# numamma/numamma

Hardware: AMD Instinct MI355X
Metric: PEBS samples/s analysed (device-resident) (higher is better)
Workload: dtype u64

## Files before the change

numamma_amd/csrc/nmg_route.hip:

```cpp
#include <algorithm>

#include "nmg_device.h"
#include "nmg_route.h"

namespace nmg {

static_assert((uint64_t)kItemChunks * kChunk * kLaneMaxWeight < (1ull << kPackShift), "packed weight per item");


struct XRec {
  uint64_t addr, ts, w;
  uint64_t loc;
  uint32_t th, acc;
  bool esc;
  __device__ __forceinline__ uint32_t g(const XLayout& xl) const { return uint32_t(loc >> xl.obits); }
  __device__ __forceinline__ uint32_t off(const XLayout& xl) const {
    return uint32_t(loc & ((1ull << xl.obits) - 1)) << 3;
  }
};

__device__ __forceinline__ uint4 x_encode(const XLayout& xl, uint64_t pb, uint64_t addr, uint64_t ts, uint64_t w,
                                          uint32_t g, uint32_t off, uint32_t th, uint32_t acc) {
  const uint64_t ar = addr - pb, tr = ts - xl.tbase;
  const bool fit = (ar >> kAddrBits) == 0 && ts >= xl.tbase && (tr >> kTsBits) == 0 && w < xl.wesc;
// ... 652 lines not shown
      }
      rt_stamp<TIMING>(rt, 5);
      bool staged = false, counts = false;
      if (__ballot(lined)) {
        lid &= kLwLineMask;
        const uint32_t j = (uint32_t)dst & 3u, S = lw_s(lw), ahead = (lid - S) & kLwLineMask;
        counts = lined && !(lw & kLwBroken) && ahead < ahead_max;
        staged = counts && ahead == 0 && dst != ~0ull;
        if (lined && !(lw & kLwBroken) && ahead >= ahead_max) atomicOr(&s_lw[X.q], kLwBroken);
        if (staged) {
          s_line[X.q * 4 + j] = X.a;
          s_ldst[X.q] = (uint32_t)(dst >> 2);
        }
        __builtin_amdgcn_fence(__ATOMIC_RELEASE, "workgroup", "local");
        LineWord o = 0;
        if (counts)
          o = atomicAdd(&s_lw[X.q], (kLwOne << (3 * (lid & (kLwAhead - 1)))) +
                                        (staged ? kLwOne << (kLwMaskShift + j) : LineWord(0)));
        const bool done = counts && lw_count(o, lid) == 3 && lw_s(o) == lid;
        const uint32_t dmask = counts ? lw_mask(o) | (staged ? 1u << j : 0u) : 0u;
        if (TIMING) rt.acc[8] += (uint64_t)__popcll(__ballot(counts && !staged));
        const uint64_t dm = __ballot(done);
        if (dm) {
          if (done)
            s_tab[wave][__popcll(dm & ((1ull << lane) - 1))] =
                make_uint2(X.q | (dmask << 11) | (lid << 16), (uint32_t)(dst >> 2));
          __builtin_amdgcn_fence(__ATOMIC_RELEASE, "wavefront", "local");
          __builtin_amdgcn_wave_barrier();
          __builtin_amdgcn_fence(__ATOMIC_ACQUIRE, "wavefront", "local");
          const uint32_t nd = (uint32_t)__popcll(dm);
          auto piece_done = [&](uint2 t, uint32_t k) {
            __builtin_amdgcn_fence(__ATOMIC_RELEASE, "workgroup", "local");
            if (k == 0) {
              const uint32_t tq = t.x & 2047u;
              uint32_t l = t.x >> 16, m = (t.x >> 11) & 15u;
              while (true) {
                const LineWord ow = atomicAdd(&s_lw[tq], (kLwOne << kLwSShift) - (LineWord(4) << (3 * (l & (kLwAhead - 1)))) -
                                                            (LineWord(m) << kLwMaskShift));
                l = (l + 1) & kLwLineMask;
                if (lw_count(ow, l) != 4) break;
                m = 0;
              }
            }
          };
          for (uint32_t j0 = 0; j0 < nd; j0 += 16) {
            const uint32_t jj = j0 + ((uint32_t)lane >> 2);
            if (jj < nd) {
              const uint2 t = s_tab[wave][jj];
              const uint32_t tq = t.x & 2047u, tm = (t.x >> 11) & 15u, k = lane & 3;
              if ((tm >> k) & 1) rec16[uint64_t(t.y) * 4 + k] = rec16_of(s_line[tq * 4 + k]);
              piece_done(t, k);
            }
          }
          __builtin_amdgcn_fence(__ATOMIC_RELEASE, "wavefront", "local");
          __builtin_amdgcn_wave_barrier();
          __builtin_amdgcn_fence(__ATOMIC_ACQUIRE, "wavefront", "local");
        }
      }
      rt_stamp<TIMING>(rt, 9);
      const bool straight = dst != ~0ull && !counts;
      const bool alone = straight || (counts && !staged && dst != ~0ull);
      if (alone) rec16[dst] = rec16_of(X.a);
      if (TIMING) {
        rt.acc[6] += (uint64_t)__popcll(__ballot(staged));
        rt.acc[7] += (uint64_t)__popcll(__ballot(straight));
      }
      if (__ballot(ovf)) {
        if (ovf) {
          const uint64_t pbq = s_pb[X.q];
          const uint32_t o = atomicAdd(rp.ovf_cnt, 1u);
          if (o < rp.ovf_cap) {
            rp.ovf16[o] = X.a;
            rp.ovfx[o] = pbq;
          } else {
            XRec xr = x_decode(rp.xl, pbq, X.a);
            if (xr.esc) x_resolve(xr, rp.xl, p.data, p.sbufs);
            direct_attribute<TL>(p, xr.addr, xr.ts, xr.w, xr.th, xr.acc, X.lvl, rp.seq0 + xr.g(rp.xl), xr.off(rp.xl),
                             xr.g(rp.xl));
          }
        }
        vm_drain();
      }
      rt_stamp<TIMING>(rt, 10);
    };

    XF X;
    do {
      front(ra, rb, X);
      back(X);
      front(rb, ra, X);
      back(X);
    } while (d0.pad != kNoBuf);

    if (TIMING && lane == 0) {
      unsigned long long* o = p.dbg + (uint64_t(blockIdx.x) * (kWG / 64) + tid / 64) * kRouteTimingWords;
      for (int k = 0; k < 9; k++) o[k] = rt.acc[k];
      o[9] = nwin;
      uint32_t nb = 0;
      if (wave == 0)
        for (uint32_t q = 0; q < nlp; q++) nb += (s_lw[q] & kLwBroken) ? 1u : 0u;
      o[10] = nb;
      o[11] = rt.acc[9];
      o[12] = rt.acc[10];
    }
  }
  racc_drain(gacc[0], s_gsums[0], lane);
  racc_drain(gacc[1], s_gsums[1], lane);
  lds_sync();
#pragma unroll
  for (uint32_t a = 0; a < 2; a++) {
    if (tid < (int)kGlobalSums && s_gsums[a][tid])
      atomicAdd(reinterpret_cast<unsigned long long*>(p.sum64 + gsum_index(a, tid)), s_gsums[a][tid]);
    if (tid < (int)kBuckets && s_gsums[a][3 + 2 * tid]) {
      atomicMin(reinterpret_cast<unsigned long long*>(p.min64 + a * kBuckets + tid), s_gmins[a][tid]);
      atomicMax(reinterpret_cast<unsigned long long*>(p.max64 + a * kBuckets + tid), s_gmaxs[a][tid]);
    }
  }
  for (uint32_t q = tid; q < P; q += kR2WG) {
    const unsigned long long st = s_state[q];
    const uint32_t f = st_cnt(st), cu = st_cur(st), nx = st_next(st);
    if (cu == kStNone) continue;
    if (cu != kStOvf) rp.cmeta[c0 + cu] = q | (min(f, kChunk) << 24);
    if (nx != kStOvf) rp.cmeta[c0 + nx] = q | ((f > kChunk ? f - kChunk : 0u) << 24);
    if (q < nlp) {
      const uint32_t m = lw_mask(s_lw[q]);
      for (uint32_t j = 0; j < 4; j++)
        if ((m >> j) & 1u) rec16[uint64_t(s_ldst[q]) * 4 + j] = rec16_of(s_line[q * 4 + j]);
    }
  }
  if (tid == 0) rp.used[blockIdx.x] = min(s_taken, capl);
}


__global__ __launch_bounds__(256) void overflow_kernel(RouteParams rp) {
  const uint32_t n = min(*rp.ovf_cnt, rp.ovf_cap);
  for (uint32_t i = blockIdx.x * 256 + threadIdx.x; i < n; i += gridDim.x * 256) {
    XRec xr = x_decode(rp.xl, rp.ovfx[i], rp.ovf16[i]);
    if (xr.esc) x_resolve(xr, rp.xl, rp.p.data, rp.p.sbufs);
    const uint32_t lvl = ((rp.p.flags & NMG_F_OBJECT_LEVELS) || rp.p.cost)
                             ? raw_mem_lvl(rp.p.data, rp.p.sbufs[xr.g(rp.xl)].offset + xr.off(rp.xl))
                             : 0u;
    direct_attribute<true>(rp.p, xr.addr, xr.ts, xr.w, xr.th, xr.acc, lvl, rp.seq0 + xr.g(rp.xl), xr.off(rp.xl),
                     xr.g(rp.xl));
  }
}


__global__ __launch_bounds__(kWG) void count_kernel(CountParams cp) {
  __shared__ uint32_t s_cnt[kMaxParts + 1];
  const ScatterParams& r = cp.sc;
  const uint32_t tid = threadIdx.x, w = blockIdx.x, P = r.nparts;
  for (uint32_t q = tid; q < P; q += kWG) s_cnt[q] = 0;
  __syncthreads();
  const uint32_t c0 = r.chunk0[w], n = r.used[w];
  constexpr uint32_t kU = 8;
  for (uint32_t b = 0; b < n; b += kU * kWG) {
    uint32_t m[kU];
#pragma unroll
    for (uint32_t u = 0; u < kU; u++) {
      const uint32_t i = b + u * kWG + tid;
      m[u] = i < n ? r.cmeta[c0 + i] : 0u;
    }
#pragma unroll
    for (uint32_t u = 0; u < kU; u++)
      if (m[u] >> 24) atomicAdd(&s_cnt[m[u] & 0xffffffu], 1u);
  }
  __syncthreads();
  uint32_t* out = const_cast<uint32_t*>(r.pcnt) + uint64_t(w) * P;
  for (uint32_t q = tid; q < P; q += kWG) out[q] = s_cnt[q];
}

constexpr uint32_t kPlanRowGroups = kWG / 64;
__global__ __launch_bounds__(kWG) void plan_cols_kernel(PlanParams r) {
  __shared__ uint32_t s_sum[kPlanRowGroups][64];
  const uint32_t tid = threadIdx.x, c = tid & 63, rg = tid >> 6;
  const uint32_t P = r.nparts, q = blockIdx.x * 64 + c;
  const uint32_t per = (r.grid + kPlanRowGroups - 1) / kPlanRowGroups, w0 = rg * per;
  constexpr uint32_t kU = 16;
  uint32_t sum = 0;
  for (uint32_t b = 0; b < per; b += kU) {
    uint32_t v[kU];
#pragma unroll
    for (uint32_t u = 0; u < kU; u++) {
      const uint32_t w = w0 + b + u;
      v[u] = (q < P && b + u < per && w < r.grid) ? r.pcnt[uint64_t(w) * P + q] : 0u;
    }
#pragma unroll
    for (uint32_t u = 0; u < kU; u++) sum += v[u];
  }
  s_sum[rg][c] = sum;
  __syncthreads();
  uint32_t run = 0;
  for (uint32_t g = 0; g < rg; g++) run += s_sum[g][c];
  for (uint32_t b = 0; b < per; b += kU) {
    uint32_t v[kU];
#pragma unroll
    for (uint32_t u = 0; u < kU; u++) {
      const uint32_t w = w0 + b + u;
      v[u] = (q < P && b + u < per && w < r.grid) ? r.pcnt[uint64_t(w) * P + q] : 0u;
    }
#pragma unroll
    for (uint32_t u = 0; u < kU; u++) {
      const uint32_t w = w0 + b + u;
      if (q < P && b + u < per && w < r.grid) r.pcnt[uint64_t(w) * P + q] = run;
      run += v[u];
    }
  }
  if (q < P && rg == kPlanRowGroups - 1) r.pbase[q] = run;
}

__global__ __launch_bounds__(kWG) void plan_kernel(PlanParams r) {
  __shared__ uint32_t s_tot[kMaxParts + 1], s_nit[kMaxParts + 1], s_wsum[2][kWG / 64];
  const int tid = threadIdx.x, lane = tid & 63, wave = tid >> 6;
  const uint32_t P = r.nparts;
  for (uint32_t q = tid; q < P; q += kWG) {
    const uint32_t run = r.pbase[q];
    s_tot[q] = run;
    s_nit[q] = (run + kItemChunks - 1) / kItemChunks;
  }
  __syncthreads();
  const uint32_t i0 = 2 * (uint32_t)tid;
  const uint32_t t0 = i0 < P ? s_tot[i0] : 0u, t1 = i0 + 1 < P ? s_tot[i0 + 1] : 0u;
  const uint32_t n0 = i0 < P ? s_nit[i0] : 0u, n1 = i0 + 1 < P ? s_nit[i0 + 1] : 0u;
  uint32_t it = t0 + t1, in = n0 + n1;
#pragma unroll
  for (int o = 1; o < 64; o <<= 1) {
    const uint32_t a = __shfl_up(it, o, 64), b = __shfl_up(in, o, 64);
    if (lane >= o) {
      it += a;
      in += b;
    }
  }
  if (lane == 63) {
    s_wsum[0][wave] = it;
    s_wsum[1][wave] = in;
  }
  __syncthreads();
  uint32_t wt = 0, wn = 0;
  for (int w2 = 0; w2 < wave; w2++) {
    wt += s_wsum[0][w2];
    wn += s_wsum[1][w2];
  }
  const uint32_t tb = wt + it - (t0 + t1), nb = wn + in - (n0 + n1);
  for (uint32_t k = 0; k < 2; k++) {
    const uint32_t q = i0 + k;
    if (q >= P) break;
    const uint32_t base = tb + (k ? t0 : 0u), ibase = nb + (k ? n0 : 0u), tot = k ? t1 : t0;
    r.pbase[q] = base;
    for (uint32_t j = 0; j * kItemChunks < tot; j++)
      r.items[ibase + j] = make_uint4(q, base + j * kItemChunks, base + min(tot, (j + 1) * kItemChunks),
                                      tot <= kItemChunks ? 1u : 0u);
  }
  if (tid == kWG - 1) {
    r.ctl[0] = wn + in;
    r.ctl[1] = 0;
    r.ctl[3] = r.ctl[2];
    r.ctl[2] = 0;
  }
}

__global__ __launch_bounds__(kWG) void scatter_kernel(ScatterParams r) {
  __shared__ uint32_t s_cnt[kMaxParts + 1];
  const uint32_t tid = threadIdx.x, w = blockIdx.x, P = r.nparts;
  const uint32_t* off = r.pcnt + uint64_t(w) * P;
  for (uint32_t q = tid; q < P; q += kWG) s_cnt[q] = r.pbase[q] + off[q];
  __syncthreads();
  const uint32_t c0 = r.chunk0[w], n = r.used[w];
  const uint32_t pc = c0 >> r.pk;
  const uint32_t voff =
      (uint32_t)((reinterpret_cast<uint64_t>(r.pieces[pc]) - r.pool0) / (kChunk * sizeof(uint4))) - (pc << r.pk);
  constexpr uint32_t kU = 8;
  for (uint32_t b = 0; b < n; b += kU * kWG) {
    uint32_t m[kU];
#pragma unroll
    for (uint32_t u = 0; u < kU; u++) {
      const uint32_t i = b + u * kWG + tid;
      m[u] = i < n ? r.cmeta[c0 + i] : 0u;
    }
#pragma unroll
    for (uint32_t u = 0; u < kU; u++) {
      if (!(m[u] >> 24)) continue;
      const uint32_t k = atomicAdd(&s_cnt[m[u] & 0xffffffu], 1u);
      const uint32_t id = c0 + b + u * kWG + tid;
      r.clist[k] = make_uint2(id | ((m[u] >> 24) << kChunkIdBits), voff + id);
    }
  }
}


constexpr uint32_t kLWG = 1024;
constexpr int kLC = 2;

template <typename T>
__device__ __forceinline__ T l2_load(const T* p) {
  return __hip_atomic_load(p, __ATOMIC_RELAXED, __HIP_MEMORY_SCOPE_AGENT);
}

__device__ __forceinline__ void lds_pair(uint4& a, uint4& b) {
  asm volatile("" : "+v"(a.x), "+v"(a.y), "+v"(a.z), "+v"(a.w), "+v"(b.x), "+v"(b.y), "+v"(b.z), "+v"(b.w));
}
__device__ __forceinline__ void lds_pair(uint2& a, uint2& b) {
  asm volatile("" : "+v"(a.x), "+v"(a.y), "+v"(b.x), "+v"(b.y));
}

__device__ __forceinline__ uint64_t entry_id(const LocalParams& lp, uint32_t pos) {
  return lp.pe_ids ? lp.pe_ids[pos] : pos;
}

__device__ __forceinline__ int32_t match_older_pos(const Params& p, uint32_t first, uint32_t count, uint64_t addr,
                                                   uint64_t ts, uint64_t& baddr, uint64_t& hist) {
  for (uint32_t j = first + 1; j < first + count; j++) {
    const uint4* r = reinterpret_cast<const uint4*>(p.chain + j);
    const uint4 ra = r[0], rb = r[1];
    if (entry_match(ra, rb, addr, ts)) {
      const uint4 rc = r[2];
      baddr = u64of(ra.x, ra.y);
      hist = u64of(rc.x, rc.y);
      return (int32_t)j;
    }
  }
  return -1;
}

template <bool INSTR, bool PACKED, bool EXTRA>
__global__ __launch_bounds__(kLWG, 1) void local_kernel(LocalParams lp) {
  __shared__ uint64_t s_keys[kPartSlots];
  __shared__ uint4 s_pn[kPartSlots];
  __shared__ uint2 s_info[kPartSlots];
  __shared__ uint4 s_dir[kPartDir];
  __shared__ uint4 s_old[kOldLds];
  __shared__ uint32_t s_oinf[kOldLds];
  __shared__ unsigned long long s_owt[2][kPartEntries];
  __shared__ unsigned long long s_first[kPartEntries];
  __shared__ uint32_t s_pg[kPartCells / 2];
  __shared__ uint32_t s_clist[kItemChunks];
  __shared__ uint32_t s_item, s_cnext, s_nfound, s_big, s_took;
  __shared__ uint4 s_nx[4];
  __shared__ uint32_t s_coff[kItemChunks];

  Params& p = lp.p;
  const int tid = threadIdx.x, lane = tid & 63;
  const uint32_t nitems = lp.ctl[0];
  const uint32_t T = p.nb_threads;
  const bool pages = (p.flags & NMG_F_PAGE_HIST) != 0;
  RTimer rt;
#pragma unroll
  for (int k = 0; k < 12; k++) rt.acc[k] = 0;
  const bool tim = INSTR && (p.flags & kDbgLocalTiming) != 0;
  const bool nowork = INSTR && (p.flags & kDbgLocalNoWork) != 0, nosearch = INSTR && (p.flags & kDbgLocalNoSearch) != 0;
  const bool noobj = INSTR && (p.flags & kDbgLocalNoObj) != 0, nopage = INSTR && (p.flags & kDbgLocalNoPage) != 0;
  auto lstamp = [&](int i) {
    if (INSTR && tim) rt_stamp<true>(rt, i);
  };
  rt.last = tim ? stamp() : 0;
  uint32_t nchunks = 0, nit = 0;
  uint64_t textra = 0;
  uint32_t nfound = 0;
  if (tid == 0) s_nfound = 0;
  for (uint32_t i = tid; i < kPartEntries; i += kLWG) {
    s_owt[0][i] = s_owt[1][i] = 0;
    s_first[i] = ~0ull;
  }
  for (uint32_t i = tid; i < kPartCells / 2; i += kLWG) s_pg[i] = 0;
  static_assert(sizeof(PartInfo) == 48, "PartInfo: three uint4");
  auto take_next = [&]() {
    uint32_t idx = 0;
    if (lane == 0) idx = atomicAdd(lp.ctl + 1, 1u);
    idx = __builtin_amdgcn_readfirstlane(idx);
    if (lane == 0) s_item = idx;
    if (idx < nitems) {
      const uint4 nx = lp.items[idx];
      const uint32_t nq = __builtin_amdgcn_readfirstlane(nx.x);
      if (lane == 0) s_nx[0] = nx;
      if (lane < 3) s_nx[1 + lane] = reinterpret_cast<const uint4*>(lp.parts + nq)[lane];
    }
  };
  if (tid < 64) take_next();
  if (tid == 0) s_took = 0;
  while (true) {
    lds_sync();
    const uint32_t it = __builtin_amdgcn_readfirstlane(s_item);
    lstamp(6);
    if (it >= nitems) break;
    nit++;
    const uint4 item = s_nx[0];
    const uint32_t q = __builtin_amdgcn_readfirstlane(item.x);
    PartInfo pi;
    {
      uint4* pw = reinterpret_cast<uint4*>(&pi);
      pw[0] = s_nx[1];
      pw[1] = s_nx[2];
      pw[2] = s_nx[3];
    }
    const uint32_t dshift = __builtin_amdgcn_readfirstlane(pi.dshift);
    {
      static_assert(kPartKeys <= kLWG && kPartDir == kLWG && kOldLds <= kLWG, "one table element per thread");
      constexpr uint32_t kClPer = (kItemChunks + kLWG - 1) / kLWG;
      const uint32_t nk = pi.nk, nold = min(pi.ne - nk, kOldLds), ncl = item.z - item.y;
      uint64_t key = 0;
      uint4 pn = make_uint4(0, 0, 0, 0), od = pn;
      uint2 inf = make_uint2(0, 0);
      uint32_t oi = 0, cl[kClPer], cf[kClPer];
      if (tid < nk) {
        key = lp.pe_keys[uint64_t(q) * kPartSlots + tid];
        pn = lp.pe_pnode[uint64_t(q) * kPartSlots + tid];
        inf = lp.pe_info[uint64_t(q) * kPartSlots + tid];
      }
      const uint4 dd = lp.pe_dir[uint64_t(q) * kPartDir + tid];
      if (tid < nold) {
        od = lp.pe_old[uint64_t(q) * kOldLds + tid];
        oi = lp.pe_oinf[uint64_t(q) * kOldLds + tid];
      }
#pragma unroll
      for (uint32_t u = 0; u < kClPer; u++) {
        const uint2 ce = tid + u * kLWG < ncl ? lp.clist[item.y + tid + u * kLWG] : make_uint2(0u, 0u);
        cl[u] = ce.x;
        cf[u] = ce.y;
      }
      if (tid < nk) {
        s_keys[tid] = key;
        s_pn[tid] = pn;
        s_info[tid] = inf;
      }
      s_dir[tid] = dd;
      if (tid < nold) {
        s_old[tid] = od;
        s_oinf[tid] = oi;
      }
#pragma unroll
      for (uint32_t u = 0; u < kClPer; u++)
        if (tid + u * kLWG < ncl) {
          s_clist[tid + u * kLWG] = cl[u];
          s_coff[tid + u * kLWG] = cf[u];
        }
    }
    if (tid == 0) {
      s_cnext = 0;
      s_took = 0;
    }
    const uint32_t ncell = (pages && pi.pages_lds) ? T * pi.span : 0u;
    const bool excl = item.w != 0 && !(INSTR && (p.flags & kDbgLocalAtomics));
    if (tid == 0) s_big = 0;
    lds_sync();
    const uint64_t k0key = u64of(__builtin_amdgcn_readfirstlane((uint32_t)s_keys[0]),
                                 __builtin_amdgcn_readfirstlane((uint32_t)(s_keys[0] >> 32)));
    lstamp(7);

    const uint32_t nl = item.z - item.y;
    auto chunk_load = [&](uint32_t l, uint4& a) {
      const uint32_t e = l < nl ? s_coff[l] : 0u;
      a = lp.pool0[uint64_t(e) * kChunk + lane];
    };
    auto process = [&](uint32_t l0, const uint4 (&a16)[kLC]) {
      uint32_t li[kLC], cw[kLC];
      bool valid[kLC];
      uint64_t addr[kLC], ts[kLC], w[kLC];
      XRec xr[kLC];
#pragma unroll
      for (int j = 0; j < kLC; j++) {
        li[j] = l0 + j;
        cw[j] = s_clist[min(li[j], nl - 1)];
      }
#pragma unroll
      for (int j = 0; j < kLC; j++) valid[j] = (uint32_t)lane < (li[j] < nl ? cw[j] >> kChunkIdBits : 0u);
      if (INSTR && tim) {
        asm volatile("s_waitcnt vmcnt(2)" ::: "memory");
        nchunks += kLC;
      }
      lstamp(0);
      if (INSTR && nowork) {
#pragma unroll
        for (int j = 0; j < kLC; j++)
          if (lane == 0 && li[j] < nl)
            lp.cmatch[cw[j] & ((1u << kChunkIdBits) - 1)] = a16[j].x ^ a16[j].y ^ a16[j].z ^ a16[j].w;
        return;
      }
      bool esc = false;
#pragma unroll
      for (int j = 0; j < kLC; j++) {
        xr[j] = x_decode_rel(lp.xl, a16[j]);
        esc |= valid[j] && xr[j].esc;
      }
      if (__ballot(esc)) {
#pragma unroll
        for (int j = 0; j < kLC; j++)
          if (valid[j] && xr[j].esc) {
            x_resolve(xr[j], lp.xl, p.data, lp.descs);
            xr[j].addr -= k0key;
          }
        vm_drain();
      }
#pragma unroll
      for (int j = 0; j < kLC; j++) {
        addr[j] = xr[j].addr;
        ts[j] = xr[j].ts;
        w[j] = valid[j] ? xr[j].w : 0ull;
      }
      lstamp(1);
      uint32_t slot[kLC], sa[kLC], sn[kLC];
      uint4 de[kLC];
#pragma unroll
      for (int j = 0; j < kLC; j++)
        slot[j] = valid[j] ? (uint32_t)min(addr[j] >> dshift, (uint64_t)(kPartDir - 1)) : 0u;
#pragma unroll
      for (int j = 0; j < kLC; j++) de[j] = s_dir[slot[j]];
      static_assert(kLC == 2, "lds_pair: two chunks");
      lds_pair(de[0], de[1]);
#pragma unroll
      for (int j = 0; j < kLC; j++) {
        const uint32_t lo = de[j].x & 1023u, n = (de[j].x >> 10) & 2047u;
        const bool inl = n && ((de[j].x >> 21) & 1u);
        const uint64_t rs64 = addr[j] - (uint64_t(slot[j]) << dshift);
        const uint32_t rs = rs64 >> 16 ? 0x10000u : (uint32_t)rs64;
        const uint32_t c = (uint32_t)((de[j].y & 0xffffu) <= rs) + (uint32_t)((de[j].y >> 16) <= rs) +
                           (uint32_t)((de[j].z & 0xffffu) <= rs) + (uint32_t)((de[j].z >> 16) <= rs) +
                           (uint32_t)((de[j].w & 0xffffu) <= rs) + (uint32_t)((de[j].w >> 16) <= rs);
        const uint32_t a = inl ? lo + min(c, n) : lo;
        const uint32_t m = !inl ? n : (c == kDirInline && n > kDirInline) ? n - kDirInline : 0u;
        sa[j] = valid[j] ? a : 0u;
        sn[j] = valid[j] ? m : 0u;
      }
      if (INSTR && tim) {
#pragma unroll
        for (int j = 0; j < kLC; j++) rt.acc[11] += (uint64_t)__popcll(__ballot(sn[j] != 0));
      }
      {
        bool more = false;
#pragma unroll
        for (int j = 0; j < kLC; j++) more |= sn[j] != 0;
        while (more) {
          uint32_t half[kLC];
          uint64_t key[kLC];
#pragma unroll
          for (int j = 0; j < kLC; j++) {
            half[j] = (sn[j] + 1) >> 1;
            key[j] = s_keys[sa[j] + half[j]];
          }
          more = false;
#pragma unroll
          for (int j = 0; j < kLC; j++) {
            const bool le = key[j] - k0key <= addr[j];
            sa[j] += le ? half[j] : 0u;
            sn[j] = le ? sn[j] - half[j] : half[j] - (uint32_t)(sn[j] != 0);
            more |= sn[j] != 0;
          }
        }
      }
      if (INSTR && tim) {
        bool any = false;
#pragma unroll
        for (int j = 0; j < kLC; j++) any |= valid[j];
        (void)__builtin_amdgcn_readfirstlane(__ballot(any));
      }
      lstamp(2);
      const uint32_t (&r)[kLC] = sa;
      int32_t erel[kLC];
      uint64_t pofs[kLC];
      uint32_t hrel[kLC], pnw[kLC], tq[kLC];
      bool older[kLC], amb[kLC];
      {
        uint4 pn[kLC];
        uint2 inf[kLC];
#pragma unroll
        for (int j = 0; j < kLC; j++) {
          pn[j] = s_pn[r[j]];
          inf[j] = s_info[r[j]];
        }
        lds_pair(pn[0], pn[1]);
        lds_pair(inf[0], inf[1]);
#pragma unroll
        for (int j = 0; j < kLC; j++) {
          tq[j] = __builtin_amdgcn_alignbit((uint32_t)(ts[j] >> 32), (uint32_t)ts[j], kPnQShift);
          const bool live = valid[j] & !(INSTR && nosearch);
          const bool in = (addr[j] >= (uint64_t)inf[j].y) & (addr[j] < (uint64_t)pn[j].x);
          amb[j] = live & (xr[j].esc | ((pn[j].w & kPnExact) != 0) | (in & ((tq[j] == pn[j].y) | (tq[j] == pn[j].z))));
          const bool hit = live & !amb[j] & in & (tq[j] > pn[j].y) & (tq[j] < pn[j].z);
          erel[j] = hit ? (int32_t)(pn[j].w & 2047u) : -1;
          pofs[j] = hit ? addr[j] - inf[j].y : 0ull;
          hrel[j] = hit ? inf[j].x : kEmpty32;
          older[j] = live & !amb[j] & !hit & ((pn[j].w & kPnOlder) != 0);
          pnw[j] = live ? pn[j].w : 0u;
        }
      }
      bool anyamb = false;
#pragma unroll
      for (int j = 0; j < kLC; j++) {
        anyamb |= amb[j];
        if (INSTR && tim) rt.acc[10] +=(uint64_t)__popcll(__ballot(amb[j]));
      }
      if (__ballot(anyamb)) {
#pragma unroll
        for (int j = 0; j < kLC; j++) {
          if (!amb[j]) continue;
          const uint64_t fa = k0key + addr[j], ft = xr[j].esc ? ts[j] : lp.xl.tbase + ts[j];
          const uint4* gq = lp.pe_nodes + (uint64_t(q) * kPartSlots + (uint32_t)r[j]) * 2;
          const uint4 na = gq[0], nb = gq[1];
          if (entry_match(na, nb, fa, ft)) {
            erel[j] = (int32_t)(s_pn[r[j]].w & 2047u);
            pofs[j] = fa - u64of(na.x, na.y);
            hrel[j] = s_info[r[j]].x;
          } else {
            older[j] = (s_pn[r[j]].w & kPnOlder) != 0;
          }
        }
        vm_drain();
      }
      bool anyold = false;
#pragma unroll
      for (int j = 0; j < kLC; j++) anyold |= older[j];
      if (__ballot(anyold)) {
#pragma unroll
        for (int j = 0; j < kLC; j++) {
          if (!older[j] || xr[j].esc || !(pnw[j] & kPnOldLds)) continue;
          const uint32_t e = pnw[j] & 2047u, base = e - (uint32_t)r[j], c = (pnw[j] >> kPnOldShift) & 2047u;
          bool glob = false;
          for (uint32_t i = 0; i < c; i++) {
            const uint4 o = s_old[base + i];
            const bool in = addr[j] >= (uint64_t)o.w && addr[j] < (uint64_t)o.x;
            if (in && (tq[j] == o.y || tq[j] == o.z)) {
              glob = true;
              break;
            }
            if (in && tq[j] > o.y && tq[j] < o.z) {
              erel[j] = (int32_t)(e + 1 + i);
              pofs[j] = addr[j] - o.w;
              hrel[j] = s_oinf[base + i];
              break;
            }
          }
          older[j] = glob;
        }
        anyold = false;
#pragma unroll
        for (int j = 0; j < kLC; j++) anyold |= older[j];
      }
      if (__ballot(anyold)) {
#pragma unroll
        for (int j = 0; j < kLC; j++) {
          if (!older[j]) continue;
          const uint64_t fa = k0key + addr[j], ft = xr[j].esc ? ts[j] : lp.xl.tbase + ts[j];
          const uint4 d = reinterpret_cast<const uint4*>(p.nodes + pi.k0 + (uint32_t)r[j])[3];
          uint64_t hist = kHistSparse, baddr = 0;
          const int32_t pos = match_older_pos(p, d.y, d.x, fa, ft, baddr, hist);
          if (pos >= 0) {
            erel[j] = pos - (int32_t)pi.e0;
            pofs[j] = fa - baddr;
            hrel[j] = hist == kHistSparse ? kEmpty32
                      : PACKED && pi.cmap != ~0u ? lp.pe_lrel[pos]
                                         : (uint32_t)(hist - pi.cb);
          }
        }
        vm_drain();
      }
      {
        uint64_t mine = 0;
        uint32_t ml = 0, mc = 0;
#pragma unroll
        for (int j = 0; j < kLC; j++) {
          const uint64_t fm = __ballot(erel[j] >= 0);
          nfound += (uint32_t)__popcll(fm);
          mine = lane == j ? fm : mine;
          ml = lane == j ? li[j] : ml;
          mc = lane == j ? cw[j] : mc;
        }
        if (lane < kLC && ml < nl) lp.cmatch[mc & ((1u << kChunkIdBits) - 1)] = mine;
      }
      lstamp(3);
#pragma unroll
      for (int j = 0; j < kLC; j++) {
        bool ok = erel[j] >= 0 && !noobj && w[j] < kLaneMaxWeight;
        if (ok) atomicAdd(&s_owt[xr[j].acc][erel[j]], (1ull << kPackShift) | w[j]);
      }
      bool anybig = false;
#pragma unroll
      for (int j = 0; j < kLC; j++) anybig |= erel[j] >= 0 && w[j] >= kLaneMaxWeight;
      if (__ballot(anybig) && !noobj) {
        if (lane == 0) s_big = 1;
#pragma unroll
        for (int j = 0; j < kLC; j++) {
          if (erel[j] < 0 || w[j] < kLaneMaxWeight) continue;
          const uint64_t e = entry_id(lp, pi.e0 + (uint32_t)erel[j]);
          atomicAdd(reinterpret_cast<unsigned long long*>(p.sum64 + objcw_index(e, xr[j].acc, 0, p.nb_entries)), 1ull);
          atomicAdd(reinterpret_cast<unsigned long long*>(p.sum64 + objcw_index(e, xr[j].acc, 1, p.nb_entries)),
                    (unsigned long long)w[j]);
        }
        vm_drain();
      }
      if (!noobj) {
        unsigned long long cur[kLC];
#pragma unroll
        for (int j = 0; j < kLC; j++) cur[j] = s_first[erel[j] >= 0 ? erel[j] : 0];
#pragma unroll
        for (int j = 0; j < kLC; j++)
          if (erel[j] >= 0 && xr[j].loc < cur[j]) atomicMin(&s_first[erel[j]], (unsigned long long)xr[j].loc);
      }
      lstamp(4);
      if (pages && !nopage) {
        uint32_t page[kLC];
        bool glob = false;
#pragma unroll
        for (int j = 0; j < kLC; j++) {
          page[j] = uint32_t(int(pofs[j] / kPageSize));
          if (erel[j] >= 0 && hrel[j] != kEmpty32 && ncell) {
            const uint32_t c = xr[j].th * pi.span + hrel[j] + page[j], sh = 16 * (c & 1);
            atomicAdd(&s_pg[c >> 1], 1u << sh);
          }
          glob |= erel[j] >= 0 && (hrel[j] == kEmpty32 || !ncell);
        }
        if (__ballot(glob)) {
#pragma unroll
          for (int j = 0; j < kLC; j++) {
            if (erel[j] < 0) continue;
            if (hrel[j] != kEmpty32 && !ncell) {
              atomicAdd(p.hist + uint64_t(xr[j].th) * p.hist_cells + pi.cb + hrel[j] + page[j], 1u);
            } else if (hrel[j] == kEmpty32) {
              const uint32_t sidx = p.entries[entry_id(lp, pi.e0 + (uint32_t)erel[j])].sidx;
              if (sidx != ~0u)
                sparse_add(p, sparse_key(sidx, xr[j].th, page[j]), lp.seq0 + xr[j].g(lp.xl), xr[j].off(lp.xl), 1u);
            }
          }
          vm_drain();
        }
      }
      lstamp(5);
      if (EXTRA) {
        const bool lev = (p.flags & NMG_F_OBJECT_LEVELS) != 0;
        const bool tlon = p.tl != nullptr;
        const bool cost = p.cost != nullptr;
        bool need[kLC], any = false;
#pragma unroll
        for (int j = 0; j < kLC; j++) {
          need[j] = valid[j] && (p.smatch != nullptr || ((lev || tlon || cost) && erel[j] >= 0));
          any |= need[j];
        }
        if (__ballot(any)) {
          uint64_t eid[kLC];
          uint32_t lvl[kLC];
          bool row[kLC];
#pragma unroll
          for (int j = 0; j < kLC; j++) {
            eid[j] = 0;
            lvl[j] = 0;
            row[j] = false;
            if (!need[j]) continue;
            const uint64_t pos = lp.descs[xr[j].g(lp.xl)].offset + xr[j].off(lp.xl);
            const bool hit = erel[j] >= 0;
            if (hit) eid[j] = entry_id(lp, pi.e0 + (uint32_t)erel[j]);
            if (p.smatch) p.smatch[pos >> 3] = hit ? (uint32_t)eid[j] + 1u : 0u;
            if ((lev || cost) && hit) {
              lvl[j] = raw_mem_lvl(p.data, pos);
              row[j] = lev;
            }
          }
          if (lev) {
#pragma unroll
            for (int j = 0; j < kLC; j++) {
              const uint32_t key = ((uint32_t)erel[j] << 15) | (xr[j].acc << 14) | lvl[j];
              const bool small = row[j] && w[j] < kLaneMaxWeight;
              uint64_t todo = __ballot(small);
              while (todo) {
                const uint32_t lead = __builtin_amdgcn_readfirstlane((uint32_t)__builtin_ctzll(todo));
                const uint32_t k = (uint32_t)__builtin_amdgcn_readlane((int)key, (int)lead);
                const bool same = small && key == k;
                const uint64_t sm = __ballot(same);
                const uint32_t ws = wave_sum_u32(same ? (uint32_t)w[j] : 0u);
                if ((uint32_t)lane == lead)
                  level_count(p, eid[j], xr[j].acc, lvl[j], ws, (unsigned long long)__popcll(sm));
                todo &= ~sm;
              }
              if (row[j] && !small) level_count(p, eid[j], xr[j].acc, lvl[j], w[j]);
            }
          }
          if (tlon) {
            uint64_t pad[kLC];
#pragma unroll
            for (int j = 0; j < kLC; j++)
              pad[j] = need[j] && erel[j] >= 0 ? p.entries[eid[j]].pad1 : kTlNone;
#pragma unroll
            for (int j = 0; j < kLC; j++) {
              const uint64_t ft = xr[j].esc ? ts[j] : lp.xl.tbase + ts[j];
              timeline_add(p, pad[j] != kTlNone,
                           timeline_cell(p, pad[j], ft, xr[j].th, uint32_t(int(pofs[j] / kPageSize))), p.tl_rounds);
            }
          }
          if (cost) {
            uint64_t hb[kLC];
#pragma unroll
            for (int j = 0; j < kLC; j++)
              hb[j] = need[j] && erel[j] >= 0 ? p.entries[eid[j]].hist : kHistSparse;
#pragma unroll
            for (int j = 0; j < kLC; j++) {
              const uint64_t v = hb[j] != kHistSparse ? cost_value(p, xr[j].acc, lvl[j], w[j]) : 0ull;
              cost_add<true>(p, v != 0,
                             uint64_t(xr[j].th) * p.hist_cells + hb[j] + uint32_t(int(pofs[j] / kPageSize)), v,
                             p.cost_rounds);
            }
          }
          vm_drain();
        }
        if (INSTR && tim) {
          const uint64_t now = stamp();
          textra += now - rt.last;
          rt.last = now;
        }
      }
    };
    uint4 A[kLC], B[kLC];
    auto grab = [&]() -> uint32_t {
      uint32_t t = 0;
      if (lane == 0) t = atomicAdd(&s_cnext, (uint32_t)kLC);
      return __builtin_amdgcn_readfirstlane(t);
    };
    uint32_t la = grab(), lb = grab();
#pragma unroll
    for (int j = 0; j < kLC; j++) chunk_load(la + j, A[j]);
#pragma unroll
    for (int j = 0; j < kLC; j++) chunk_load(lb + j, B[j]);
    while (la < nl) {
      process(la, A);
      la = grab();
#pragma unroll
      for (int j = 0; j < kLC; j++) chunk_load(la + j, A[j]);
      if (lb < nl) process(lb, B);
      lb = grab();
#pragma unroll
      for (int j = 0; j < kLC; j++) chunk_load(lb + j, B[j]);
    }
    uint32_t won = 0;
    if (lane == 0) won = atomicExch(&s_took, 1u) == 0 ? 1u : 0u;
    if (__builtin_amdgcn_readfirstlane(won)) take_next();
    lds_sync();
    lstamp(9);
    const bool clean =excl && lp.fresh && __builtin_amdgcn_readfirstlane(lp.ctl[3]) == 0;
    const bool clean_obj = clean && __builtin_amdgcn_readfirstlane(s_big) == 0;
    for (uint32_t i = tid; i < pi.ne; i += kLWG) {
      const uint64_t e = entry_id(lp, pi.e0 + i);
#pragma unroll
      for (uint32_t a = 0; a < 2; a++) {
        const uint64_t v = s_owt[a][i];
        if (!v) continue;
        s_owt[a][i] = 0;
        const uint64_t cnt = v >> kPackShift, wt = v & ((1ull << kPackShift) - 1);
        uint64_t* pc = p.sum64 + objcw_index(e, a, 0, p.nb_entries);
        uint64_t* pw = p.sum64 + objcw_index(e, a, 1, p.nb_entries);
        if (clean_obj) {
          *pc = cnt;
          if (wt) *pw = wt;
        } else if (excl) {
          *pc = l2_load(pc) + cnt;
          if (wt) *pw = l2_load(pw) + wt;
        } else {
          atomicAdd(reinterpret_cast<unsigned long long*>(pc), (unsigned long long)cnt);
          if (wt) atomicAdd(reinterpret_cast<unsigned long long*>(pw), (unsigned long long)wt);
        }
      }
      const uint64_t floc = s_first[i];
      if (floc != ~0ull) {
        s_first[i] = ~0ull;
        const uint64_t fo = ((lp.seq0 + (floc >> lp.xl.obits)) << 32) | ((floc & ((1ull << lp.xl.obits) - 1)) << 3);
        uint64_t* pf = p.min64 + kFirstBase + e;
        if (clean) *pf = fo;
        else if (excl) *pf = min(l2_load(pf), fo);
        else atomicMin(reinterpret_cast<unsigned long long*>(pf), (unsigned long long)fo);
      }
    }
    {
      const uint32_t nw = (ncell + 1) / 2, span = pi.span;
      const uint32_t cmap = PACKED ? __builtin_amdgcn_readfirstlane(pi.cmap) : ~0u;
      const uint32_t smag = span > 1 ? 0xffffffffu / span + 1u : 0u;
      constexpr uint32_t kU = 4;
      for (uint32_t j0 = tid; j0 < nw; j0 += kU * kLWG) {
        uint32_t cnt[kU][2], old[kU][2];
        uint32_t* pc[kU][2];
#pragma unroll
        for (uint32_t u = 0; u < kU; u++) {
          const uint32_t j = j0 + u * kLWG;
          const uint32_t v = j < nw ? s_pg[j] : 0u;
          if (v) s_pg[j] = 0;
#pragma unroll
          for (uint32_t h = 0; h < 2; h++) {
            cnt[u][h] = (v >> (16 * h)) & 0xffffu;
            const uint32_t li = 2 * j + h, th = span == 1 ? li : __umulhi(li, smag), rel = li - th * span;
            uint64_t cell = pi.cb + rel;
            if (cmap != ~0u) cell = cnt[u][h] ? lp.pe_cmap[cmap + rel] : 0u;
            pc[u][h] = p.hist + uint64_t(th) * p.hist_cells + cell;
            old[u][h] = (excl && !clean && cnt[u][h]) ? l2_load(pc[u][h]) : 0u;
          }
        }
#pragma unroll
        for (uint32_t u = 0; u < kU; u++)
#pragma unroll
          for (uint32_t h = 0; h < 2; h++) {
            if (!cnt[u][h]) continue;
            if (excl) *pc[u][h] = old[u][h] + cnt[u][h];
            else atomicAdd(pc[u][h], cnt[u][h]);
          }
      }
    }
    lds_sync();
    lstamp(8);
  }
  if (lane == 0 && nfound) atomicAdd(&s_nfound, nfound);
  lds_sync();
  if (tid == 0 && s_nfound) atomicAdd(p.found, (unsigned long long)s_nfound);
  if (INSTR && tim && lane == 0) {
    unsigned long long* o = p.dbg + (uint64_t(blockIdx.x) * (kWG / 64) + tid / 64) * kRouteTimingWords;
    for (int k = 0; k < 9; k++) o[k] = rt.acc[k];
    o[9] = nchunks;
    o[10] = nit;
    o[11] = rt.acc[9];
    o[12] = rt.acc[10];
    o[13] = rt.acc[11];
    o[14] = textra;
  }
}


__global__ __launch_bounds__(kWG) void found_kernel(FoundParams r) {
  __shared__ uint32_t s_found[kFoundLds];
  const int tid = threadIdx.x, lane = tid & 63;
  const uint32_t w = blockIdx.x;
  const uint32_t g0 = r.ranges[w], nbuf = r.ranges[w + 1] - g0, nl = min(nbuf, kFoundLds);
  for (uint32_t i = tid; i < nl; i += kWG) s_found[i] = 0;
  __syncthreads();
  const uint64_t k0 = uint64_t(r.chunk0[w]) * kChunk, k1 = k0 + uint64_t(r.used[w]) * kChunk;
  const uint64_t gmask = (1ull << r.gbits) - 1;
  const NMG_GLOBAL uint64_t* const xwords = (const NMG_GLOBAL uint64_t*)pool_vbase(r.pieces, r.pk, r.chunk0[w]);
  constexpr int kU = 4;
  for (uint64_t k = k0 + tid; k < k1; k += kU * kWG) {
    uint64_t bits[kU], xw[kU];
#pragma unroll
    for (int u = 0; u < kU; u++) {
      const uint64_t kk = k + u * kWG;
      bits[u] = kk < k1 && (r.cmeta[kk / kChunk] >> 24) ? r.cmatch[kk / kChunk] : 0ull;
      xw[u] = ((bits[u] >> lane) & 1) ? xwords[2 * kk + 1] >> r.gshift : 0ull;
    }
#pragma unroll
    for (int u = 0; u < kU; u++) {
      if (!((bits[u] >> lane) & 1)) continue;
      const uint32_t g = (uint32_t)(xw[u] & gmask);
      if (g - g0 < nl) atomicAdd(&s_found[g - g0], 1u);
      else atomicAdd(r.bufcnt + r.nb_bufs + g, 1u);
    }
  }
  __syncthreads();
  for (uint32_t i = tid; i < nl; i += kWG)
    if (s_found[i]) atomicAdd(r.bufcnt + r.nb_bufs + g0 + i, s_found[i]);
}


hipError_t launch_route(uint32_t grid, hipStream_t s, const RouteParams& r) {
  const bool timing = (r.p.flags & kDbgRouteTiming) != 0, tl = r.p.tl != nullptr || r.p.cost != nullptr;
  if (timing && tl) hipLaunchKernelGGL((route2_kernel<true, true>), dim3(grid), dim3(kR2WG), 0, s, r);
  else if (timing) hipLaunchKernelGGL((route2_kernel<true, false>), dim3(grid), dim3(kR2WG), 0, s, r);
  else if (tl) hipLaunchKernelGGL((route2_kernel<false, true>), dim3(grid), dim3(kR2WG), 0, s, r);
  else hipLaunchKernelGGL((route2_kernel<false, false>), dim3(grid), dim3(kR2WG), 0, s, r);
  return hipGetLastError();
}

hipError_t launch_plan(hipStream_t s, const PlanParams& r) {
  if (r.nparts) hipLaunchKernelGGL(plan_cols_kernel, dim3((r.nparts + 63) / 64), dim3(kWG), 0, s, r);
  hipLaunchKernelGGL(plan_kernel, dim3(1), dim3(kWG), 0, s, r);
  return hipGetLastError();
}

hipError_t launch_overflow(hipStream_t s, const RouteParams& r) {
  hipLaunchKernelGGL(overflow_kernel, dim3(1024), dim3(256), 0, s, r);
  return hipGetLastError();
}

hipError_t launch_count(uint32_t grid, hipStream_t s, const CountParams& r) {
  hipLaunchKernelGGL(count_kernel, dim3(grid), dim3(kWG), 0, s, r);
  return hipGetLastError();
}

hipError_t launch_scatter(uint32_t grid, hipStream_t s, const ScatterParams& r) {
  hipLaunchKernelGGL(scatter_kernel, dim3(grid), dim3(kWG), 0, s, r);
  return hipGetLastError();
}

template <bool INSTR, bool PACKED>
static void launch_local_as(bool extra, uint32_t grid, hipStream_t s, const LocalParams& r) {
  if (extra) hipLaunchKernelGGL((local_kernel<INSTR, PACKED, true>), dim3(grid), dim3(kLWG), 0, s, r);
  else hipLaunchKernelGGL((local_kernel<INSTR, PACKED, false>), dim3(grid), dim3(kLWG), 0, s, r);
}

hipError_t launch_local(uint32_t grid, hipStream_t s, const LocalParams& r) {
  constexpr uint32_t kInstr = kDbgLocalTiming | kDbgLocalNoWork | kDbgLocalNoSearch | kDbgLocalNoObj |
                              kDbgLocalNoPage | kDbgLocalAtomics;
  const bool instr = (r.p.flags & kInstr) != 0, packed = r.pe_cmap != nullptr;
  const bool extra = (r.p.flags & NMG_F_OBJECT_LEVELS) != 0 || r.p.smatch != nullptr || r.p.tl != nullptr ||
                     r.p.cost != nullptr;
  if (packed) {
    if (instr) launch_local_as<true, true>(extra, grid, s, r);
    else launch_local_as<false, true>(extra, grid, s, r);
  } else {
    if (instr) launch_local_as<true, false>(extra, grid, s, r);
    else launch_local_as<false, false>(extra, grid, s, r);
  }
  return hipGetLastError();
}

hipError_t launch_found(uint32_t grid, hipStream_t s, const FoundParams& r) {
  hipLaunchKernelGGL(found_kernel, dim3(grid), dim3(kWG), 0, s, r);
  return hipGetLastError();
}

}
```

Baseline: 48.54 billion.

## Reload rare-path kernel args from kernarg segment; speculate first old-LDS probe

Rare branches (escape resolve, ambiguous match, older-chain search, big weights, global hist, extras) now re-read the kernel arguments they need straight from the kernarg segment, rather than keeping them live in scalar registers across the main loop. This is meant to lower SGPR/VGPR pressure in the hot loop. The older-LDS search also loads the first candidate for both lanes' items without branching, resolves it with predicated selects, and only falls back to the serial loop when more candidates remain. The cost is extra scalar loads on the rare paths and an unconditional LDS read per item.

```diff
diff --git a/numamma_amd/csrc/nmg_route.hip b/numamma_amd/csrc/nmg_route.hip
--- a/numamma_amd/csrc/nmg_route.hip
+++ b/numamma_amd/csrc/nmg_route.hip
@@ -978,15 +978,31 @@
 __device__ __forceinline__ void lds_pair(uint2& a, uint2& b) {
   asm volatile("" : "+v"(a.x), "+v"(a.y), "+v"(b.x), "+v"(b.y));
 }
-
-__device__ __forceinline__ uint64_t entry_id(const LocalParams& lp, uint32_t pos) {
-  return lp.pe_ids ? lp.pe_ids[pos] : pos;
-}
-
-__device__ __forceinline__ int32_t match_older_pos(const Params& p, uint32_t first, uint32_t count, uint64_t addr,
-                                                   uint64_t ts, uint64_t& baddr, uint64_t& hist) {
+__device__ __forceinline__ void lds_pair(uint32_t& a, uint32_t& b) { asm volatile("" : "+v"(a), "+v"(b)); }
+
+#define NMG_KAS __attribute__((address_space(4)))
+typedef const NMG_KAS LocalParams* KArgs;
+__device__ __forceinline__ KArgs rare_args() {
+  KArgs k = (KArgs)__builtin_amdgcn_kernarg_segment_ptr();
+  asm volatile("" : "+s"(k));
+  return k;
+}
+template <typename T>
+__device__ __forceinline__ T karg(const NMG_KAS T* f) {
+  T v;
+  __builtin_memcpy(&v, f, sizeof(T));
+  return v;
+}
+
+__device__ __forceinline__ uint64_t entry_id(const uint32_t* pe_ids, uint32_t pos) {
+  return pe_ids ? pe_ids[pos] : pos;
+}
+__device__ __forceinline__ uint64_t entry_id(const LocalParams& lp, uint32_t pos) { return entry_id(lp.pe_ids, pos); }
+
+__device__ __forceinline__ int32_t match_older_pos(const DevEntry* chain, uint32_t first, uint32_t count,
+                                                   uint64_t addr, uint64_t ts, uint64_t& baddr, uint64_t& hist) {
   for (uint32_t j = first + 1; j < first + count; j++) {
-    const uint4* r = reinterpret_cast<const uint4*>(p.chain + j);
+    const uint4* r = reinterpret_cast<const uint4*>(chain + j);
     const uint4 ra = r[0], rb = r[1];
     if (entry_match(ra, rb, addr, ts)) {
       const uint4 rc = r[2];
@@ -1158,10 +1174,14 @@
         esc |= valid[j] && xr[j].esc;
       }
       if (__ballot(esc)) {
+        const KArgs ka = rare_args();
+        const XLayout rxl = karg(&ka->xl);
+        const uint8_t* rdata = ka->p.data;
+        const BufDesc* rdescs = ka->descs;
 #pragma unroll
         for (int j = 0; j < kLC; j++)
           if (valid[j] && xr[j].esc) {
-            x_resolve(xr[j], lp.xl, p.data, lp.descs);
+            x_resolve(xr[j], rxl, rdata, rdescs);
             xr[j].addr -= k0key;
           }
         vm_drain();
@@ -1265,11 +1285,14 @@
         if (INSTR && tim) rt.acc[10] +=(uint64_t)__popcll(__ballot(amb[j]));
       }
       if (__ballot(anyamb)) {
+        const KArgs ka = rare_args();
+        const uint64_t tbase = ka->xl.tbase;
+        const uint4* pe_nodes = ka->pe_nodes;
 #pragma unroll
         for (int j = 0; j < kLC; j++) {
           if (!amb[j]) continue;
-          const uint64_t fa = k0key + addr[j], ft = xr[j].esc ? ts[j] : lp.xl.tbase + ts[j];
-          const uint4* gq = lp.pe_nodes + (uint64_t(q) * kPartSlots + (uint32_t)r[j]) * 2;
+          const uint64_t fa = k0key + addr[j], ft = xr[j].esc ? ts[j] : tbase + ts[j];
+          const uint4* gq = pe_nodes + (uint64_t(q) * kPartSlots + (uint32_t)r[j]) * 2;
           const uint4 na = gq[0], nb = gq[1];
           if (entry_match(na, nb, fa, ft)) {
             erel[j] = (int32_t)(s_pn[r[j]].w & 2047u);
@@ -1285,44 +1308,78 @@
 #pragma unroll
       for (int j = 0; j < kLC; j++) anyold |= older[j];
       if (__ballot(anyold)) {
+        bool use[kLC], more[kLC], anymore = false;
+        uint32_t ob[kLC], oi[kLC];
+        uint4 o[kLC];
 #pragma unroll
         for (int j = 0; j < kLC; j++) {
-          if (!older[j] || xr[j].esc || !(pnw[j] & kPnOldLds)) continue;
-          const uint32_t e = pnw[j] & 2047u, base = e - (uint32_t)r[j], c = (pnw[j] >> kPnOldShift) & 2047u;
-          bool glob = false;
-          for (uint32_t i = 0; i < c; i++) {
-            const uint4 o = s_old[base + i];
-            const bool in = addr[j] >= (uint64_t)o.w && addr[j] < (uint64_t)o.x;
-            if (in && (tq[j] == o.y || tq[j] == o.z)) {
-              glob = true;
-              break;
+          use[j] = older[j] & !xr[j].esc & ((pnw[j] & kPnOldLds) != 0);
+          ob[j] = use[j] ? (pnw[j] & 2047u) - (uint32_t)r[j] : 0u;
+        }
+#pragma unroll
+        for (int j = 0; j < kLC; j++) {
+          o[j] = s_old[ob[j]];
+          oi[j] = s_oinf[ob[j]];
+        }
+        lds_pair(o[0], o[1]);
+        lds_pair(oi[0], oi[1]);
+#pragma unroll
+        for (int j = 0; j < kLC; j++) {
+          const bool in = (addr[j] >= (uint64_t)o[j].w) & (addr[j] < (uint64_t)o[j].x);
+          const bool glob = use[j] & in & ((tq[j] == o[j].y) | (tq[j] == o[j].z));
+          const bool hit = use[j] & in & (tq[j] > o[j].y) & (tq[j] < o[j].z);
+          erel[j] = hit ? (int32_t)((pnw[j] & 2047u) + 1) : erel[j];
+          pofs[j] = hit ? addr[j] - o[j].w : pofs[j];
+          hrel[j] = hit ? oi[j] : hrel[j];
+          more[j] = use[j] & !glob & !hit & (((pnw[j] >> kPnOldShift) & 2047u) > 1);
+          older[j] = use[j] ? glob : older[j];
+          anymore |= more[j];
+        }
+        if (__ballot(anymore)) {
+#pragma unroll
+          for (int j = 0; j < kLC; j++) {
+            if (!more[j]) continue;
+            const uint32_t e = pnw[j] & 2047u, base = e - (uint32_t)r[j], c = (pnw[j] >> kPnOldShift) & 2047u;
+            bool glob = false;
+            for (uint32_t i = 1; i < c; i++) {
+              const uint4 on = s_old[base + i];
+              const bool in = addr[j] >= (uint64_t)on.w && addr[j] < (uint64_t)on.x;
+              if (in && (tq[j] == on.y || tq[j] == on.z)) {
+                glob = true;
+                break;
+              }
+              if (in && tq[j] > on.y && tq[j] < on.z) {
+                erel[j] = (int32_t)(e + 1 + i);
+                pofs[j] = addr[j] - on.w;
+                hrel[j] = s_oinf[base + i];
+                break;
+              }
             }
-            if (in && tq[j] > o.y && tq[j] < o.z) {
-              erel[j] = (int32_t)(e + 1 + i);
-              pofs[j] = addr[j] - o.w;
-              hrel[j] = s_oinf[base + i];
-              break;
-            }
-          }
-          older[j] = glob;
+            older[j] = glob;
+          }
         }
         anyold = false;
 #pragma unroll
         for (int j = 0; j < kLC; j++) anyold |= older[j];
       }
       if (__ballot(anyold)) {
+        const KArgs ka = rare_args();
+        const uint64_t tbase = ka->xl.tbase;
+        const DevEntry* nodes = ka->p.nodes;
+        const DevEntry* chain = ka->p.chain;
+        const uint32_t* pe_lrel = ka->pe_lrel;
 #pragma unroll
         for (int j = 0; j < kLC; j++) {
           if (!older[j]) continue;
-          const uint64_t fa = k0key + addr[j], ft = xr[j].esc ? ts[j] : lp.xl.tbase + ts[j];
-          const uint4 d = reinterpret_cast<const uint4*>(p.nodes + pi.k0 + (uint32_t)r[j])[3];
+          const uint64_t fa = k0key + addr[j], ft = xr[j].esc ? ts[j] : tbase + ts[j];
+          const uint4 d = reinterpret_cast<const uint4*>(nodes + pi.k0 + (uint32_t)r[j])[3];
           uint64_t hist = kHistSparse, baddr = 0;
-          const int32_t pos = match_older_pos(p, d.y, d.x, fa, ft, baddr, hist);
+          const int32_t pos = match_older_pos(chain, d.y, d.x, fa, ft, baddr, hist);
           if (pos >= 0) {
             erel[j] = pos - (int32_t)pi.e0;
             pofs[j] = fa - baddr;
             hrel[j] = hist == kHistSparse ? kEmpty32
-                      : PACKED && pi.cmap != ~0u ? lp.pe_lrel[pos]
+                      : PACKED && pi.cmap != ~0u ? pe_lrel[pos]
                                          : (uint32_t)(hist - pi.cb);
           }
         }
@@ -1352,12 +1409,16 @@
       for (int j = 0; j < kLC; j++) anybig |= erel[j] >= 0 && w[j] >= kLaneMaxWeight;
       if (__ballot(anybig) && !noobj) {
         if (lane == 0) s_big = 1;
+        const KArgs ka = rare_args();
+        const uint32_t* pe_ids = ka->pe_ids;
+        uint64_t* sum64 = ka->p.sum64;
+        const uint32_t nb_entries = ka->p.nb_entries;
 #pragma unroll
         for (int j = 0; j < kLC; j++) {
           if (erel[j] < 0 || w[j] < kLaneMaxWeight) continue;
-          const uint64_t e = entry_id(lp, pi.e0 + (uint32_t)erel[j]);
-          atomicAdd(reinterpret_cast<unsigned long long*>(p.sum64 + objcw_index(e, xr[j].acc, 0, p.nb_entries)), 1ull);
-          atomicAdd(reinterpret_cast<unsigned long long*>(p.sum64 + objcw_index(e, xr[j].acc, 1, p.nb_entries)),
+          const uint64_t e = entry_id(pe_ids, pi.e0 + (uint32_t)erel[j]);
+          atomicAdd(reinterpret_cast<unsigned long long*>(sum64 + objcw_index(e, xr[j].acc, 0, nb_entries)), 1ull);
+          atomicAdd(reinterpret_cast<unsigned long long*>(sum64 + objcw_index(e, xr[j].acc, 1, nb_entries)),
                     (unsigned long long)w[j]);
         }
         vm_drain();
@@ -1384,15 +1445,20 @@
           glob |= erel[j] >= 0 && (hrel[j] == kEmpty32 || !ncell);
         }
         if (__ballot(glob)) {
+          const KArgs ka = rare_args();
+          const Params rp = karg(&ka->p);
+          const XLayout rxl = karg(&ka->xl);
+          const uint32_t* pe_ids = ka->pe_ids;
+          const uint64_t seq0 = ka->seq0;
 #pragma unroll
           for (int j = 0; j < kLC; j++) {
             if (erel[j] < 0) continue;
             if (hrel[j] != kEmpty32 && !ncell) {
-              atomicAdd(p.hist + uint64_t(xr[j].th) * p.hist_cells + pi.cb + hrel[j] + page[j], 1u);
+              atomicAdd(rp.hist + uint64_t(xr[j].th) * rp.hist_cells + pi.cb + hrel[j] + page[j], 1u);
             } else if (hrel[j] == kEmpty32) {
-              const uint32_t sidx = p.entries[entry_id(lp, pi.e0 + (uint32_t)erel[j])].sidx;
+              const uint32_t sidx = rp.entries[entry_id(pe_ids, pi.e0 + (uint32_t)erel[j])].sidx;
               if (sidx != ~0u)
-                sparse_add(p, sparse_key(sidx, xr[j].th, page[j]), lp.seq0 + xr[j].g(lp.xl), xr[j].off(lp.xl), 1u);
+                sparse_add(rp, sparse_key(sidx, xr[j].th, page[j]), seq0 + xr[j].g(rxl), xr[j].off(rxl), 1u);
             }
           }
           vm_drain();
@@ -1410,6 +1476,11 @@
           any |= need[j];
         }
         if (__ballot(any)) {
+          const KArgs ka = rare_args();
+          const Params rp = karg(&ka->p);
+          const XLayout rxl = karg(&ka->xl);
+          const BufDesc* rdescs = ka->descs;
+          const uint32_t* pe_ids = ka->pe_ids;
           uint64_t eid[kLC];
           uint32_t lvl[kLC];
           bool row[kLC];
@@ -1419,12 +1490,12 @@
             lvl[j] = 0;
             row[j] = false;
             if (!need[j]) continue;
-            const uint64_t pos = lp.descs[xr[j].g(lp.xl)].offset + xr[j].off(lp.xl);
+            const uint64_t pos = rdescs[xr[j].g(rxl)].offset + xr[j].off(rxl);
             const bool hit = erel[j] >= 0;
-            if (hit) eid[j] = entry_id(lp, pi.e0 + (uint32_t)erel[j]);
-            if (p.smatch) p.smatch[pos >> 3] = hit ? (uint32_t)eid[j] + 1u : 0u;
+            if (hit) eid[j] = entry_id(pe_ids, pi.e0 + (uint32_t)erel[j]);
+            if (rp.smatch) rp.smatch[pos >> 3] = hit ? (uint32_t)eid[j] + 1u : 0u;
             if ((lev || cost) && hit) {
-              lvl[j] = raw_mem_lvl(p.data, pos);
+              lvl[j] = raw_mem_lvl(rp.data, pos);
               row[j] = lev;
             }
           }
@@ -1441,35 +1512,35 @@
                 const uint64_t sm = __ballot(same);
                 const uint32_t ws = wave_sum_u32(same ? (uint32_t)w[j] : 0u);
                 if ((uint32_t)lane == lead)
-                  level_count(p, eid[j], xr[j].acc, lvl[j], ws, (unsigned long long)__popcll(sm));
+                  level_count(rp, eid[j], xr[j].acc, lvl[j], ws, (unsigned long long)__popcll(sm));
                 todo &= ~sm;
               }
-              if (row[j] && !small) level_count(p, eid[j], xr[j].acc, lvl[j], w[j]);
+              if (row[j] && !small) level_count(rp, eid[j], xr[j].acc, lvl[j], w[j]);
             }
           }
           if (tlon) {
             uint64_t pad[kLC];
 #pragma unroll
             for (int j = 0; j < kLC; j++)
-              pad[j] = need[j] && erel[j] >= 0 ? p.entries[eid[j]].pad1 : kTlNone;
+              pad[j] = need[j] && erel[j] >= 0 ? rp.entries[eid[j]].pad1 : kTlNone;
 #pragma unroll
             for (int j = 0; j < kLC; j++) {
-              const uint64_t ft = xr[j].esc ? ts[j] : lp.xl.tbase + ts[j];
-              timeline_add(p, pad[j] != kTlNone,
-                           timeline_cell(p, pad[j], ft, xr[j].th, uint32_t(int(pofs[j] / kPageSize))), p.tl_rounds);
+              const uint64_t ft = xr[j].esc ? ts[j] : rxl.tbase + ts[j];
+              timeline_add(rp, pad[j] != kTlNone,
+                           timeline_cell(rp, pad[j], ft, xr[j].th, uint32_t(int(pofs[j] / kPageSize))), rp.tl_rounds);
             }
           }
           if (cost) {
             uint64_t hb[kLC];
 #pragma unroll
             for (int j = 0; j < kLC; j++)
-              hb[j] = need[j] && erel[j] >= 0 ? p.entries[eid[j]].hist : kHistSparse;
+              hb[j] = need[j] && erel[j] >= 0 ? rp.entries[eid[j]].hist : kHistSparse;
 #pragma unroll
             for (int j = 0; j < kLC; j++) {
-              const uint64_t v = hb[j] != kHistSparse ? cost_value(p, xr[j].acc, lvl[j], w[j]) : 0ull;
-              cost_add<true>(p, v != 0,
-                             uint64_t(xr[j].th) * p.hist_cells + hb[j] + uint32_t(int(pofs[j] / kPageSize)), v,
-                             p.cost_rounds);
+              const uint64_t v = hb[j] != kHistSparse ? cost_value(rp, xr[j].acc, lvl[j], w[j]) : 0ull;
+              cost_add<true>(rp, v != 0,
+                             uint64_t(xr[j].th) * rp.hist_cells + hb[j] + uint32_t(int(pofs[j] / kPageSize)), v,
+                             rp.cost_rounds);
             }
           }
           vm_drain();
```

Measured after the change: 48.53 billion. Within noise of the previous version (-0.0%).
